# linjonathan/tropical_cyclone_risk

Hardware: AMD Instinct MI355X
Metric: storm-steps/sec (100k-storm ensemble) (higher is better)
Workload: dtype f64

## Files before the change

### tropical_cyclone_risk_amd/csrc/tcr_abi.hip

```cpp
#include <hip/hip_runtime.h>

#include <atomic>
#include <chrono>
#include <cmath>
#include <condition_variable>
#include <memory>
#include <mutex>
#include <thread>
#include <type_traits>
#include <cstdio>
#include <cstdlib>
#include <cstring>
#include <string>
#include <vector>

#include "tcr_kernels.hip"
#include "tcr_seed.hip"
#include "tcr_compact.hip"
#include "tcr_prep.hip"
#include "tcr_thermo.hip"
#ifdef TCR_EXPERIMENTS
#include "tcr_experiments.h"
#endif

// ... 136 lines not shown
    size_t vrec_cap = 0;
    unsigned long long *d_tiles = nullptr;
    size_t tiles_cap = 0;
    unsigned long long *d_queue = nullptr;
    uint16_t *d_sidx = nullptr;
    size_t sidx_cap = 0;
    double *d_park[2] = {nullptr, nullptr};
    size_t park_cap[2] = {0, 0};
    double2 *d_sc_table = nullptr;
    double *d_tab = nullptr;
    int tab_np = 0, tab_ns = 0;
    double2 *d_pf = nullptr;
    size_t pf_cap = 0;
    int fs_period = 0;
    int cu_count = 256;
    uint8_t *d_screen_skip = nullptr;
    size_t screen_skip_cap = 0;
    int32_t *d_und_list = nullptr;
    size_t und_list_cap = 0;
    unsigned long long *d_und_count = nullptr;
    float *d_stat32 = nullptr;
    bool stat32_stale = true;
    int32_t *d_tc_idx = nullptr;
    size_t tc_idx_cap = 0;
    int64_t *d_tc_count = nullptr;
    double *d_cell = nullptr; size_t cell_cap = 0; int cell_bins = 0;
    bool cell_counts_open = false;
    unsigned int *d_hist_partial = nullptr;
    uint8_t *d_probe = nullptr;
    int probe_cap = 0;
    int storms_per_lane = 1;
    tcr_tune tune;
    double *h_stage[2] = {nullptr, nullptr};
    size_t h_stage_cap = 0;
    hipEvent_t h_stage_ev[2] = {nullptr, nullptr};
// ... 578 lines not shown
template <typename R>
int integrate_impl(tcr_ctx *ctx, const tcr_storms *in, const TracksT<R> out, void *stream_, uint64_t *stats = nullptr,
                   const int64_t *stats_n_dev = nullptr, int64_t n_expected = 0)
{
    HIPCHK(ctx, hipSetDevice(ctx->device));
    const int64_t n = in->n;
    if (n < 0) return fail(ctx, "tcr_integrate: negative n");
    if (n == 0) return 0;
    hipStream_t st = stream_ ? (hipStream_t)stream_ : ctx->stream;
    const tcr_params &P = ctx->prm;
    const size_t ns = (size_t)P.n_steps;
    constexpr size_t REC = (size_t)step_rec_doubles<R>();
    if (grow(ctx, &ctx->d_fs, &ctx->fs_cap, ((size_t)n * ns * 4 * sizeof(R) + 7) / 8)) return -1;
    const int max_rk = P.max_rk_steps > 0 ? P.max_rk_steps : 64;
    if (grow(ctx, &ctx->d_srec, &ctx->srec_cap, (size_t)n * max_rk * REC)) return -1;
    if (grow(ctx, &ctx->d_vrec, &ctx->vrec_cap, (size_t)n * max_rk * kVRec)) return -1;
    if (max_rk > 65535) return fail(ctx, "tcr_params.max_rk_steps must be <= 65535");
    {
        double *p = reinterpret_cast<double *>(ctx->d_sidx);
        if (grow(ctx, &p, &ctx->sidx_cap, ((size_t)n * ns * sizeof(uint16_t) + 7) / 8)) { ctx->d_sidx = nullptr; return -1; }
        ctx->d_sidx = reinterpret_cast<uint16_t *>(p);
    }
    R *fs = reinterpret_cast<R *>(ctx->d_fs);
    EvalKT<R> EK{};
    bool affine = false;
    if (eval_k_ready<R>(ctx, EK, &affine, st)) return -1;

    hipEvent_t *ev = nullptr;
    if (ctx->timing && !ctx->capturing && timing_events(ctx, &ev)) return -1;
    if (ev) HIPCHK(ctx, hipEventRecord(ev[0], st));
    const int wps = std::is_same<R, double>::value ? TCR_INT_WPS : TCR_INT_WPS_F32;
    unsigned waves = integrate_waves(ctx, (n_expected > 0 && n_expected < n) ? n_expected : n, wps);
    const int thr = park_threshold(ctx, waves, wps);
    const unsigned final_waves = park_final_waves(ctx);
    const bool segmented = kFsMfmaColGroups == 2 && thr > 0 && waves > final_waves && kMaxPasses > 1 && fourier_on_matrix_cores(ctx) &&
                           (int)P.n_steps > kFsSegSamples + 16 && ctx->tune.table_segments != 0;
    int prune_sample = -1;
    if (out.tc_rows_only && ctx->tune.prune != 0) {
        const double t2d = 2 * 86400.0, step_out = P.total_time / (double)(P.n_steps - 1);
        const int j = (int)floor(t2d / step_out);
        if (j >= 1 && j < P.n_steps - 1 && ts_host(P, j) == t2d) {
            prune_sample = j;
            double *q = reinterpret_cast<double *>(ctx->d_screen_skip);
            if (grow(ctx, &q, &ctx->screen_skip_cap, ((size_t)n + 7) / 8)) { ctx->d_screen_skip = nullptr; return -1; }
            ctx->d_screen_skip = reinterpret_cast<uint8_t *>(q);
            double *u = reinterpret_cast<double *>(ctx->d_und_list);
            if (grow(ctx, &u, &ctx->und_list_cap, ((size_t)n + 1) / 2 + 1)) { ctx->d_und_list = nullptr; return -1; }
            ctx->d_und_list = reinterpret_cast<int32_t *>(u);
            if (!ctx->d_und_count && dev_alloc(ctx, &ctx->d_und_count, (size_t)1)) return -1;
        }
    }
    {
        BatchReset z{};
        z.queue = ctx->d_queue; z.queue_words = (int)kQueueWords;
        if (prune_sample >= 0) { z.und_count = ctx->d_und_count; z.flags = out.flags; z.n_flags = n; }
        if (out.tc_rows_only) z.tc_count = reinterpret_cast<unsigned long long *>(ctx->d_tc_count);
        if (launch_fourier<R>(ctx, n, in->n_dev, in->phases, fs, st, segmented ? kFsFirst : kFsAll, nullptr, nullptr, &z)) return -1;
    }
    STAGE(TCR_STAGE_FOURIER);
    if (ev) HIPCHK(ctx, hipEventRecord(ev[1], st));
    {
        KArgsT<R> a{};
        a.P = P; a.D = dev_fields(ctx); a.K = EK; a.n = n; a.n_dev = in->n_dev;
        a.lon0 = in->lon0; a.lat0 = in->lat0; a.v0 = in->v0; a.m0 = in->m0; a.h_bl = in->h_bl;
        a.slot = in->slot; a.phases = in->phases; a.fs = fs; a.srec = ctx->d_srec; a.vrec = ctx->d_vrec; a.max_rk_steps = max_rk;
        a.n_valid = out.n_valid; a.status = out.status; a.nfev = out.nfev;
        a.n_accept = out.n_accept; a.n_reject = out.n_reject;
        a.queue = ctx->d_queue;
        a.prune_sample = prune_sample;
        a.screen_skip = prune_sample >= 0 ? ctx->d_screen_skip : nullptr;
        if (prune_sample >= 0) {
            a.und_list = ctx->d_und_list; a.und_count = ctx->d_und_count;
        }
        const size_t park_items = segmented ? (size_t)n : (size_t)waves * kWave;
        if (thr > 0 && grow(ctx, &ctx->d_park[0], &ctx->park_cap[0], park_items * kParkRec)) return -1;
        if (thr > 0 && grow(ctx, &ctx->d_park[1], &ctx->park_cap[1], park_items * kParkRec)) return -1;
        const bool probe = std::is_same<R, double>::value && ctx->d_probe;
        if (probe) { a.probe = ctx->d_probe; a.probe_cap = ctx->probe_cap; }
        bool seg_events = false;
        for (int pass = 0; pass < kMaxPasses; ++pass) {
            const bool last = thr <= 0 || waves <= final_waves || pass == kMaxPasses - 1;
            a.pass = pass;
            a.fill_pct = pass_fill_pct();
            a.threshold = last ? 0 : thr;
            a.park_in = ctx->d_park[(pass + 1) & 1];
            a.park_out = ctx->d_park[pass & 1];
            a.t_limit = (segmented && pass == 0) ? ts_host(P, kFsSegSamples - 2) : 1e300;
// ... 2 lines not shown
            if (segmented && pass == 0) {
                if (ev) HIPCHK(ctx, hipEventRecord(ev[4], st));
                if (launch_fourier<R>(ctx, n, in->n_dev, in->phases, fs, st, kFsRest, ctx->d_park[0], ctx->d_queue + kMaxPasses)) return -1;
                if (ev) HIPCHK(ctx, hipEventRecord(ev[5], st));
                seg_events = true;
                continue;
            }
            waves = (unsigned)(((size_t)waves * (size_t)(thr - 1) + kWave - 1) / kWave);
        }
        if (ev && !seg_events) { HIPCHK(ctx, hipEventRecord(ev[4], st)); HIPCHK(ctx, hipEventRecord(ev[5], st)); }
    }
    STAGE(TCR_STAGE_INTEGRATE);
    if (ev) HIPCHK(ctx, hipEventRecord(ev[2], st));
    {
        EArgsT<R> a{};
        a.P = P; a.D = dev_fields(ctx); a.n = n; a.n_dev = in->n_dev; a.max_rk_steps = max_rk; a.srec = ctx->d_srec; a.vrec = ctx->d_vrec; a.fs = fs;
        a.slot = in->slot; a.n_valid = out.n_valid; a.status = out.status; a.n_accept = out.n_accept;
        a.lon = out.lon; a.lat = out.lat; a.v = out.v; a.m = out.m; a.vmax = out.vmax;
        a.envw = out.envw; a.flags = out.flags; a.pad_state = out.pad_state;
        a.K = EK;
        a.screen_skip = prune_sample >= 0 ? ctx->d_screen_skip : nullptr;
        if (prune_sample >= 0) { a.und_list = ctx->d_und_list; a.und_count = ctx->d_und_count; }
        const unsigned chunks = (unsigned)((ns + kPostThreads - 1) / kPostThreads);
        if (out.tc_rows_only) {
            if ((size_t)n > ctx->tc_idx_cap) {
                if (ctx->d_tc_idx) HIPCHK(ctx, hipFree(ctx->d_tc_idx));
                ctx->d_tc_idx = nullptr; ctx->tc_idx_cap = 0;
                if (dev_alloc(ctx, &ctx->d_tc_idx, (size_t)n)) return -1;
                ctx->tc_idx_cap = (size_t)n;
            }
            a.tc_list = ctx->d_tc_idx; a.tc_count = reinterpret_cast<unsigned long long *>(ctx->d_tc_count);
            hipLaunchKernelGGL(k_screen<R>, dim3((unsigned)((n + kScreenStorms - 1) / kScreenStorms)), dim3(kScreenThreads), 0, st, a);
            STAGE(TCR_STAGE_SCREEN);
            STAGE(TCR_STAGE_SELECT_TC);
            a.list = ctx->d_tc_idx; a.count = ctx->d_tc_count;
        }
        int64_t cap = kEmitGridCap;
        if (ctx->tune.emit_grid_cap > 0) cap = ctx->tune.emit_grid_cap;
        const unsigned gx = (out.tc_rows_only && n > 2 * cap) ? (unsigned)cap : (unsigned)n;
        hipLaunchKernelGGL(k_dense<R>, dim3(gx), dim3(kWave), 0, st, a, ctx->d_sidx);
        STAGE(TCR_STAGE_DENSE);
        const unsigned ex = gx;
        if (out.tc_rows_only) {
            if (affine) hipLaunchKernelGGL((k_emit<R, true, false>), dim3(ex, chunks), dim3(kPostThreads), 0, st, a, ctx->d_sidx);
            else hipLaunchKernelGGL((k_emit<R, false, false>), dim3(ex, chunks), dim3(kPostThreads), 0, st, a, ctx->d_sidx);
            if ((int64_t)ex < n) {
                a.item_base = ex;
// ... 71 lines not shown
        (void)hipFree(g->d_lon); (void)hipFree(g->d_lat); (void)hipFree(g->d_rlon); (void)hipFree(g->d_rlat);
        (void)hipFree(g->d_lon32); (void)hipFree(g->d_lat32); (void)hipFree(g->d_rlon32); (void)hipFree(g->d_rlat32);
    }
    for (auto &s : ctx->slots) { (void)hipFree(s.wind); (void)hipFree(s.thermo); (void)hipFree(s.rh); (void)hipFree(s.wind32); (void)hipFree(s.thermo32); }
    (void)hipFree(ctx->d_stat32); (void)hipFree(ctx->d_land); (void)hipFree(ctx->d_bathy); (void)hipFree(ctx->d_land32); (void)hipFree(ctx->d_bathy32);
    (void)hipFree(ctx->d_slots); (void)hipFree(ctx->d_stat); (void)hipFree(ctx->d_mask_bits); (void)hipFree(ctx->d_nstat); (void)hipFree(ctx->d_nbathy);
    (void)hipFree(ctx->d_fs); (void)hipFree(ctx->d_srec); (void)hipFree(ctx->d_vrec);
    for (auto &ev : ctx->ev_pool) if (ev) (void)hipEventDestroy(ev);
    for (auto &ev : ctx->st_pool) if (ev) (void)hipEventDestroy(ev);
    for (auto &g : ctx->graphs) { if (g.exec) (void)hipGraphExecDestroy(g.exec); if (g.graph) (void)hipGraphDestroy(g.graph); }
    (void)hipFree(ctx->d_round_key);
    ctx->hz.release(); ctx->wf.release(); ctx->ls.release();
    (void)hipFree(ctx->lf_xy); (void)hipFree(ctx->lf_bits);
    (void)hipFree(ctx->d_cl);
    for (int i = 0; i < 2; ++i) { if (ctx->h_stage[i]) (void)hipHostFree(ctx->h_stage[i]); if (ctx->h_stage_ev[i]) (void)hipEventDestroy(ctx->h_stage_ev[i]); }
    (void)hipFree(ctx->d_hist_partial); (void)hipFree(ctx->d_cell); (void)hipFree(ctx->d_tiles); (void)hipFree(ctx->d_tc_idx); (void)hipFree(ctx->d_tc_count); (void)hipFree(ctx->d_queue); (void)hipFree(ctx->d_sidx); (void)hipFree(ctx->d_park[0]); (void)hipFree(ctx->d_park[1]); (void)hipFree(ctx->d_sc_table); (void)hipFree(ctx->d_pf); (void)hipFree(ctx->d_screen_skip); (void)hipFree(ctx->d_und_list); (void)hipFree(ctx->d_und_count); (void)hipFree(ctx->d_tab);
    (void)hipStreamDestroy(ctx->stream);
    delete ctx;
    return 0;
}

int tcr_params_set(tcr_ctx *ctx, const tcr_params *p)
{
    if (!ctx || !p) return -1;
    if (p->n_series < 1 || p->n_series > TCR_MAX_SERIES) return fail(ctx, "n_series out of range");
    if (p->n_steps < 2 || p->n_steps > 4096) return fail(ctx, "n_steps must be in [2, 4096]");
    if (p->max_rk_steps < 0 || p->max_rk_steps > 4096) return fail(ctx, "max_rk_steps out of range");
    if (!(p->total_time > 0) || !(p->dt_out > 0)) return fail(ctx, "total_time and dt_out must be positive");
    ctx->prm = *p;
    ctx->have_prm = true;
    ++ctx->epoch;
// ... 1181 lines not shown
```

### tropical_cyclone_risk_amd/csrc/tcr_device.h

```cpp
#pragma once
#include <hip/hip_runtime.h>
#include <stdint.h>

#include <type_traits>

#include "../../include/tcrisk_hip.h"

#define RD(x) (x)

#ifndef TCR_FUSE
#define TCR_FUSE 1
#endif
#ifndef TCR_FAST_DIV
#define TCR_FAST_DIV 1
#endif
#ifndef TCR_FAST_SQRT
#define TCR_FAST_SQRT 1
#endif
#ifndef TCR_SHARE_COS
#define TCR_SHARE_COS 1
#endif
#ifndef TCR_FAST_POW
#define TCR_FAST_POW 1
#endif
// ... 295 lines not shown
template <typename R> struct Widths;
template <> struct Widths<double> { static constexpr int W = 2, T = 2, H = 2, F = 2; };
template <> struct Widths<float> { static constexpr int W = 4, T = 4, H = 2, F = 4; };

__device__ __forceinline__ double ts_at(const tcr_params &P, int i)
{
    return (i == P.n_steps - 1) ? P.total_time : (double)i * (P.total_time / (double)(P.n_steps - 1));
}

template <typename R>
__device__ __forceinline__ double ts_k(const EvalKT<R> &K, int i)
{
    return (i == RD(K.n_steps) - 1) ? RD(K.total_time) : (double)i * RD(K.tstep);
}

struct FsBracket {
    int lo;
    double x_lo, dx;
};

template <typename R>
__device__ __forceinline__ FsBracket fs_bracket(const EvalKT<R> &K, double t)
{
    const int ns = RD(K.n_steps);
    int idx = (int)ceil(t * RD(K.inv_tstep));
    idx = idx < 0 ? 0 : (idx > ns - 1 ? ns - 1 : idx);
    const bool dn = (idx > 0) && (ts_k(K, idx - 1) >= t);
    const bool up = !dn && (idx < ns - 1) && (ts_k(K, idx) < t);
    idx += up ? 1 : (dn ? -1 : 0);
    idx = idx < 1 ? 1 : idx;
// ... 373 lines not shown
```

### tropical_cyclone_risk_amd/csrc/tcr_kernels.hip

```cpp
#include "tcr_device.h"

namespace tcr {

template <typename R>
struct KArgsT {
    tcr_params P;
    DevFields D;
    EvalKT<R> K;
    int64_t n;
    const int64_t *n_dev;
    const double *lon0, *lat0, *v0, *m0, *h_bl;
    const int32_t *slot;
    const double *phases;
    R *fs;
    double *srec;
    int32_t *n_valid, *status, *nfev, *n_accept, *n_reject;
    unsigned long long *queue;
    int max_rk_steps;
    int pass;
    int threshold;
    int fill_pct;
    const double *park_in;
    double *park_out;
    double t_limit;
    uint8_t *probe;
    int probe_cap;
    double *vrec;
    int prune_sample;
    uint8_t *screen_skip;
    int32_t *und_list;
    unsigned long long *und_count;
};
using KArgs = KArgsT<double>;
constexpr int kVRec = 12;
constexpr int kMaxPasses = 16;
constexpr int kParkRec = 18;

__device__ __forceinline__ int64_t n_eff(int64_t n, const int64_t *n_dev)
{
    if (!n_dev) return n;
    const int64_t m = *n_dev;
    return m < n ? m : n;
}

template <typename R>
__device__ __forceinline__ void store_fs(R *__restrict__ dst, double a, double b, double c, double d)
{
    typedef typename VecT<R, 4>::type V4;
    V4 v; v[0] = (R)a; v[1] = (R)b; v[2] = (R)c; v[3] = (R)d;
    *reinterpret_cast<V4 *>(dst) = v;
}
// ... 104 lines not shown
#endif
constexpr int kFsMfmaColTiles = TCR_FS_MFMA_TILES;
#ifndef TCR_FS_MFMA_WAVES
#define TCR_FS_MFMA_WAVES 2
#endif
constexpr int kFsMfmaWaves = TCR_FS_MFMA_WAVES;
constexpr int kFsMfmaColGroups = 24 / (kFsMfmaWaves * kFsMfmaColTiles);
constexpr int kFsMfmaWgsPerCu = TCR_FS_MFMA_WPS;
static_assert(kFsMfmaColGroups * kFsMfmaWaves * kFsMfmaColTiles == 24, "column tiles per wave must be 6, 3, 2 or 1");
constexpr int kFsMfmaKSteps = 8;
constexpr int kFsMfmaMaxSamples = 24 * 16;

struct BatchReset {
    unsigned long long *queue;
    int queue_words;
    unsigned long long *und_count;
    int32_t *flags;
    int64_t n_flags;
    unsigned long long *tc_count;
};
__device__ __forceinline__ void batch_reset(const BatchReset &z, int64_t i, int64_t stride)
{
    if (!z.queue) return;
    for (int64_t k = i; k < z.queue_words; k += stride) z.queue[k] = 0ull;
    if (i == 0 && z.und_count) *z.und_count = 0ull;
    if (i == 0 && z.tc_count) *z.tc_count = 0ull;
    for (int64_t k = i; k < z.n_flags; k += stride) z.flags[k] = 0;
}
__global__ __launch_bounds__(256) void k_batch_reset(BatchReset z)
{
    batch_reset(z, (int64_t)blockIdx.x * 256 + threadIdx.x, (int64_t)gridDim.x * 256);
}

__global__ __launch_bounds__(256) void k_phase_factors_frag(tcr_params P, int64_t n, const int64_t *__restrict__ n_dev,
                                                            const double *__restrict__ phases, double *__restrict__ frag,
                                                            const int64_t *__restrict__ list, const unsigned long long *__restrict__ list_count,
                                                            BatchReset z)
{
    batch_reset(z, (int64_t)blockIdx.x * 256 + threadIdx.x, (int64_t)gridDim.x * 256);
    const int N = P.n_series;
// ... 137 lines not shown
#define A30 (44. / 45)
#define A31 (-56. / 15)
#define A32 (32. / 9)
#define A40 (19372. / 6561)
#define A41 (-25360. / 2187)
#define A42 (64448. / 6561)
#define A43 (-212. / 729)
#define A50 (9017. / 3168)
#define A51 (-355. / 33)
#define A52 (46732. / 5247)
#define A53 (49. / 176)
#define A54 (-5103. / 18656)
__device__ constexpr double RK_C[7] = {0, 1. / 5, 3. / 10, 4. / 5, 8. / 9, 1, 1};
__device__ constexpr double RK_B[6] = {35. / 384, 0, 500. / 1113, 125. / 192, -2187. / 6784, 11. / 84};
__device__ constexpr double RK_E[7] = {-71. / 57600, 0, 71. / 16695, -71. / 1920, 17253. / 339200, -22. / 525, 1. / 40};
__device__ constexpr double RK_P[7][4] = {
    {1, -8048581381. / 2820520608, 8663915743. / 2820520608, -12715105075. / 11282082432},
    {0, 0, 0, 0},
    {0, 131558114200. / 32700410799, -68118460800. / 10900136933, 87487479700. / 32700410799},
    {0, -1754552775. / 470086768, 14199869525. / 1410260304, -10690763975. / 1880347072},
    {0, 127303824393. / 49829197408, -318862633887. / 49829197408, 701980252875. / 199316789632},
    {0, -282668133. / 205662961, 2019193451. / 616988883, -1453857185. / 822651844},
    {0, 40617522. / 29380423, -110615467. / 29380423, 69997945. / 29380423}};

__device__ __forceinline__ double rms4(double a, double b, double c, double d)
{
    TCR_FP_FUSE_RK
    return qsqrt<double>(a * a + b * b + c * c + d * d) / 2.0;
}

__device__ __forceinline__ int samples_upto(const tcr_params &P, double t_emit)
{
    const int ns = P.n_steps;
    int k = (int)(t_emit / (P.total_time / (double)(ns - 1)));
    k = k < 0 ? 0 : (k > ns - 1 ? ns - 1 : k);
    while (k + 1 < ns && ts_at(P, k + 1) <= t_emit) ++k;
    while (k >= 0 && ts_at(P, k) > t_emit) --k;
    return k + 1;
// ... 38 lines not shown
    __syncthreads();
    const int ns = P.n_steps;
    const double tb = P.total_time;
    constexpr int REC = step_rec_doubles<R>();
    typedef typename VecT<R, 4>::type V4;
#define KS(j, i) Kl[((j) * 4 + (i)) * kWave + lane]

    long long sid = -1;
    int status = kRunning, nfev = 0, nacc = 0, nrej = 0, next_out = 0;
    bool active = false, fresh = false, exhausted = false, rejected = false;
    const R *wind = nullptr, *thermo = nullptr;
    const R *fs = nullptr;
    double *srec = nullptr;
    R ck_h = R(0.0);
    int cur_slot = 0;
    bool doomed = false;
    R y[4] = {0, 0, 0, 0}, f[4] = {0, 0, 0, 0}, yn[4] = {0, 0, 0, 0};
    R e[4] = {0, 0, 0, 0};
    double et = 0;
    double t = 0, h = 0, ha = 0, h_abs = 0, t_new = 0;
    R g = R(0.0);
    CornerCacheT<R> CC;
    cache_reset(CC);
    RhsPipeT<R, AFFINE, SM> PIPE;
    double etn = 0;

    auto finalize = [&]() {
        a.n_valid[sid] = next_out;
        a.status[sid] = status;
        a.nfev[sid] = (status == TCR_STATUS_GATED) ? 0 : nfev;
        a.n_accept[sid] = nacc;
        a.n_reject[sid] = nrej;
        if (a.screen_skip) a.screen_skip[sid] = doomed ? 1 : 0;
        if (a.und_list && !doomed && status != TCR_STATUS_GATED && next_out > 0)
            a.und_list[atomicAdd(a.und_count, 1ull)] = (int32_t)sid;
        active = false;
    };
    auto attempt_setup = [&]() {
        const double min_step = 10 * fabs(nextafter(t, INFINITY) - t);
        if (ha < min_step) { status = TCR_STATUS_STEP_FAIL; finalize(); return; }
        h = ha;
        t_new = t + h;
        if (t_new - tb > 0) t_new = tb;
        h = t_new - t;
        ha = fabs(h);
        for (int i = 0; i < 4; ++i) {
            KS(0, i) = f[i];
            const R dy = R(0.0) + f[i] * R(A10);
            e[i] = y[i] + dy * (R)h;
        }
// ... 5 lines not shown
        if (ha > P.max_step) ha = P.max_step;
        else if (ha < min_step) ha = min_step;
        rejected = false;
        attempt_setup();
    };

    auto park = [&](unsigned long long mask) {
        const int leader = __ffsll((long long)mask) - 1;
        unsigned long long base = 0;
        if (lane == leader) base = atomicAdd(a.queue + kMaxPasses + a.pass, (unsigned long long)__popcll(mask));
        base = __shfl(base, leader);
        if ((mask >> lane) & 1ull) {
            const size_t item = (size_t)(base + (unsigned long long)__popcll(mask & ((1ull << lane) - 1ull)));
            double2 *o = reinterpret_cast<double2 *>(a.park_out + item * kParkRec);
            const long long c0 = (long long)(unsigned)nfev | ((long long)nacc << 32);
            const long long c1 = (long long)(unsigned)nrej | ((long long)(doomed ? 1 : 0) << 30) | ((long long)(rejected ? 1 : 0) << 31) | ((long long)next_out << 32);
            o[0] = make_double2(t, h); o[1] = make_double2(t_new, ha); o[2] = make_double2((double)g, (double)y[0]);
            o[3] = make_double2((double)y[1], (double)y[2]); o[4] = make_double2((double)y[3], (double)f[0]);
            o[5] = make_double2((double)f[1], (double)f[2]);
            o[6] = make_double2((double)f[3], __longlong_as_double(sid));
            o[7] = make_double2(__longlong_as_double(c0), __longlong_as_double(c1));
            o[8] = make_double2((double)ck_h, __longlong_as_double((long long)cur_slot));
        }
    };
    __shared__ unsigned long long occ[4];
    if (lane == 0) { occ[0] = 0; occ[1] = 0; occ[2] = wall_clock64(); occ[3] = clock64(); }
    for (;;) {
        {
            const unsigned long long late = __ballot(active && t_new > a.t_limit);
            if (late) { park(late); if ((late >> lane) & 1ull) active = false; }
        }
// ... 2 lines not shown
            const int leader = __ffsll((long long)want) - 1;
            unsigned long long base = 0;
            if (lane == leader) base = atomicAdd(q_head, (unsigned long long)__popcll(want));
            base = __shfl(base, leader);
            if (!active && !exhausted) {
                const long long item = (long long)(base + (unsigned long long)__popcll(want & ((1ull << lane) - 1ull)));
                if (item >= n_items) {
                    exhausted = true;
                } else {
                    int slot_id;
                    if (a.pass == 0) {
                        sid = item;
                        const double lo0 = a.lon0[sid], la0 = a.lat0[sid], vv0 = a.v0[sid], mm0 = a.m0[sid], hb0 = a.h_bl[sid];
                        slot_id = a.slot[sid];
                        y[0] = (R)lo0; y[1] = (R)la0; y[2] = (R)vv0; y[3] = (R)mm0; ck_h = ck_over_h<R>(K, (R)hb0);
                        status = kRunning; nfev = 0; nacc = 0; nrej = 0; next_out = 0; doomed = false;
                        t = 0.0;
                        et = 0.0; e[0] = y[0]; e[1] = y[1]; e[2] = y[2]; e[3] = y[3];
                        fresh = true;
                    } else {
                        const double2 *r = reinterpret_cast<const double2 *>(a.park_in + (size_t)item * kParkRec);
                        const double2 r0 = r[0], r1 = r[1], r2 = r[2], r3 = r[3], r4 = r[4], r5 = r[5], r6 = r[6], r7 = r[7], r8 = r[8];
                        t = r0.x; h = r0.y; t_new = r1.x; ha = r1.y; g = (R)r2.x;
                        y[0] = (R)r2.y; y[1] = (R)r3.x; y[2] = (R)r3.y; y[3] = (R)r4.x;
                        f[0] = (R)r4.y; f[1] = (R)r5.x; f[2] = (R)r5.y; f[3] = (R)r6.x;
                        sid = __double_as_longlong(r6.y);
                        const long long c0 = __double_as_longlong(r7.x), c1 = __double_as_longlong(r7.y);
                        nfev = (int)(c0 & 0xffffffffll); nacc = (int)(c0 >> 32);
                        nrej = (int)(c1 & 0x3fffffffll); doomed = (c1 >> 30) & 1; rejected = (c1 >> 31) & 1; next_out = (int)(c1 >> 32);
                        ck_h = (R)r8.x; slot_id = (int)__double_as_longlong(r8.y);
                        status = kRunning;
                        for (int i = 0; i < 4; ++i) {
                            KS(0, i) = f[i];
                            const R dy = R(0.0) + f[i] * R(A10);
                            e[i] = y[i] + dy * (R)h;
                        }
                        et = t + RK_C[1] * h;
                        fresh = false;
                    }
                    if (slot_id < kIntSlotCache) { wind = s_wind[slot_id]; thermo = s_thermo[slot_id]; }
                    else { const DevSlot S = D.slots[slot_id]; wind = slot_wind<R>(S); thermo = slot_thermo<R>(S); }
                    cur_slot = slot_id;
                    fs = a.fs + sid * ns * 4;
                    srec = a.srec + sid * (long long)a.max_rk_steps * REC;
// ... 58 lines not shown
                    et = etn;
                } else {
                    double er[4];
                    for (int i = 0; i < 4; ++i) {
                        const double sc = P.atol + fmax(fabs((double)y[i]), fabs((double)yn[i])) * P.rtol;
                        double acc = 0.0;
                        for (int j = 0; j < 7; ++j) acc += (double)KS(j, i) * RK_E[j];
                        er[i] = qdiv_nz<double>(acc * h, sc);
                    }
                    const double err = rms4(er[0], er[1], er[2], er[3]);
                    const double pw = 0.9 * inv_fifth_root<double>(err);
                    if (err < 1) {
                        double fac = (err == 0) ? 10.0 : fmin(10.0, pw);
                        if (rejected && fac > 1) fac = 1;
                        ha *= fac;
                        if (nacc < a.max_rk_steps && !doomed) {
                            double *rec = srec + (size_t)nacc * REC;
                            double2 *o = reinterpret_cast<double2 *>(rec);
                            o[0] = make_double2(t, h);
                            o[1] = make_double2(t_new, 0.0);
                            V4 *body = reinterpret_cast<V4 *>(rec + kStepHdr);
                            V4 v; v[0] = y[0]; v[1] = y[1]; v[2] = y[2]; v[3] = y[3];
                            body[0] = v;
                            for (int j = 0; j < 7; ++j) {
                                V4 kk; kk[0] = KS(j, 0); kk[1] = KS(j, 1); kk[2] = KS(j, 2); kk[3] = KS(j, 3);
                                body[1 + j] = kk;
                            }
                            double2 *vr = reinterpret_cast<double2 *>(a.vrec + (sid * (long long)a.max_rk_steps + nacc) * kVRec);
                            vr[0] = make_double2(t, h);
                            vr[1] = make_double2(t_new, (double)y[2]);
                            vr[2] = make_double2((double)KS(0, 2), (double)KS(1, 2));
                            vr[3] = make_double2((double)KS(2, 2), (double)KS(3, 2));
                            vr[4] = make_double2((double)KS(4, 2), (double)KS(5, 2));
                            vr[5] = make_double2((double)KS(6, 2), 0.0);
                        }
                        ++nacc;
                        const double t_old = t;
                        t = t_new;
                        const R v_old = y[2];
                        for (int i = 0; i < 4; ++i) { y[i] = yn[i]; f[i] = r.d[i]; }
                        h_abs = ha;
                        if (t - tb >= 0) status = TCR_STATUS_FINISHED;
                        const R g_new = event_fn<R>(P, y[0], y[1], y[2]);
                        double t_emit = t;
                        if (g == R(0.0)) { status = TCR_STATUS_EVENT; t_emit = t_old; }
                        else if (g_new == R(0.0)) status = TCR_STATUS_EVENT;
                        g = g_new;
                        const int first_out = next_out;
                        next_out = samples_upto(P, t_emit);
                        int s2d = -1;
                        if (a.prune_sample >= 0 && !doomed) {
                            if (first_out <= a.prune_sample && a.prune_sample < next_out) s2d = a.prune_sample;
                            else if (status != kRunning && next_out <= a.prune_sample && first_out < next_out) s2d = next_out - 1;
                        }
                        if (s2d >= 0) {
                            TCR_FP_EXACT
                            R Qv[4];
                            for (int k = 0; k < 4; ++k) {
                                R acc = R(0.0);
                                for (int q = 0; q < 7; ++q) acc += KS(q, 2) * R(RK_P[q][k]);
                                Qv[k] = acc;
                            }
                            const R x = (R)((ts_at(P, s2d) - t_old) / h);
                            const R p1 = x, p2 = p1 * x, p3 = p2 * x, p4 = p3 * x;
                            R acc = R(0.0);
                            acc += Qv[0] * p1; acc += Qv[1] * p2; acc += Qv[2] * p3; acc += Qv[3] * p4;
                            const R v2d = (R)h * acc + v_old;
                            doomed = !((double)v2d >= P.v_2d_thresh);
                        }
                        if (status == kRunning && !doomed && nacc >= a.max_rk_steps) status = TCR_STATUS_STEP_OVERFLOW;
                        if (status != kRunning) finalize();
                        else begin_step();
                    } else {
                        ha *= fmax(0.2, pw);
                        rejected = true;
                        ++nrej;
                        attempt_setup();
                    }
                }
            } else if (live && slot == 0) {
                const R sdu = r.w[0] - r.w[2], sdw = r.w[1] - r.w[3];
                const R shear = sqrt(sdu * sdu + sdw * sdw);
                if (r.vpot > R(0) && shear * r.chi / r.vpot >= R(1)) {
                    status = TCR_STATUS_GATED;
                    finalize();
// ... 44 lines not shown
    DevFields D;
    int64_t n;
    const int64_t *n_dev;
    int max_rk_steps;
    const double *srec;
    const double *vrec;
    const R *fs;
    const int32_t *slot;
    const int32_t *n_valid, *status, *n_accept;
    R *lon, *lat, *v, *m, *vmax, *envw;
    int32_t *flags;
    const int32_t *pad_state;
    const int32_t *list;
    const int64_t *count;
    int64_t item_base;
    const uint8_t *screen_skip;
    const int32_t *und_list;
    const unsigned long long *und_count;
    int32_t *tc_list;
    unsigned long long *tc_count;
    EvalKT<R> K;
};
using EArgs = EArgsT<double>;
static_assert(sizeof(EvalKT<double>) % 8 == 0 && sizeof(EvalKT<float>) % 8 == 0, "EvalK is copied to LDS in eight-byte words");
constexpr int kBitAny15 = 1 << 8, kBitVmax = 1 << 9;
constexpr int kBitListed = 1 << 10;
#ifndef TCR_POST_THREADS
#define TCR_POST_THREADS 128
#endif
constexpr int kPostThreads = TCR_POST_THREADS;
#ifndef TCR_EMIT_GRID_CAP
#define TCR_EMIT_GRID_CAP 8192
#endif
// ... 190 lines not shown
            }
        }
    } while (LIST && (item += gridDim.x) < n_items);
}

constexpr int kScreenThreads = 256;
constexpr int kScreenGroup = 16;
constexpr int kScreenStorms = kScreenThreads / kScreenGroup;

template <typename R>
__global__ __launch_bounds__(kScreenThreads, TCR_SHADOW_WPS) void k_screen(EArgsT<R> a)
{
    __shared__ R cap[kScreenStorms][3];
    const tcr_params &P = a.P;
    const int g = threadIdx.x / kScreenGroup, l = threadIdx.x % kScreenGroup;
    const int64_t item = (int64_t)blockIdx.x * kScreenStorms + g;
    if (a.und_list && (int64_t)blockIdx.x * kScreenStorms >= (int64_t)*a.und_count) return;
    const bool listed = a.und_list && item < (int64_t)*a.und_count;
    const int64_t sid = a.und_list ? (listed ? (int64_t)a.und_list[item] : 0) : item;
    const bool on = a.und_list ? listed : sid < a.n;
    const bool exists = a.und_list ? listed : sid < n_eff(a.n, a.n_dev);
    const int ns = P.n_steps;
    int n = 0, nst = 0, st = TCR_STATUS_GATED;
    if (exists) {
        n = a.n_valid[sid]; nst = a.n_accept[sid]; st = a.status[sid];
        nst = nst < a.max_rk_steps ? nst : a.max_rk_steps;
        if (a.screen_skip && a.screen_skip[sid]) n = 0;
    }
    const double step_out = P.total_time / (double)(ns - 1);
    const double t2d = 2 * 86400.0;
    const bool clamp2d = n > 0 && t2d >= ts_at(P, n - 1);
    const int j2d = clamp2d ? n - 1 : (int)floor(t2d / step_out);
    bool any15 = false;
    const double *vrec_storm = a.vrec + sid * (int64_t)a.max_rk_steps * kVRec;
    struct StepV {
        double t_old, h64;
        R hh, y0, Q[4];
        int i_lo, i_hi;
    };
    auto load_step = [&](int j) {
        const double2 *rj = reinterpret_cast<const double2 *>(vrec_storm + (size_t)j * kVRec);
        const double2 r0 = rj[0], r1 = rj[1], r2 = rj[2], r3 = rj[3], r4 = rj[4], r5 = rj[5];
        StepV s;
        s.t_old = r0.x; s.h64 = r0.y;
        const double t_new = r1.x;
        s.hh = (R)s.h64; s.y0 = (R)r1.y;
        const R kq[7] = {(R)r2.x, (R)r2.y, (R)r3.x, (R)r3.y, (R)r4.x, (R)r4.y, (R)r5.x};
        for (int k = 0; k < 4; ++k) {
            R acc = R(0.0);
            for (int q = 0; q < 7; ++q) acc += kq[q] * R(RK_P[q][k]);
            s.Q[k] = acc;
        }
        s.i_lo = (j == 0) ? 0 : samples_upto(P, s.t_old);
        s.i_hi = samples_upto(P, t_new);
        s.i_hi = s.i_hi < n ? s.i_hi : n;
        return s;
    };
    auto v_at = [&](const StepV &s, int i) -> R {
        const R x = (R)((ts_at(P, i) - s.t_old) / s.h64);
        const R p1 = x, p2 = p1 * x, p3 = p2 * x, p4 = p3 * x;
        R acc = R(0.0);
        acc += s.Q[0] * p1; acc += s.Q[1] * p2; acc += s.Q[2] * p3; acc += s.Q[3] * p4;
        return s.hh * acc + s.y0;
    };
    auto caps = [&](const StepV &s) {
        if (s.i_lo <= j2d && j2d < s.i_hi) cap[g][0] = v_at(s, j2d);
        if (s.i_lo <= j2d + 1 && j2d + 1 < s.i_hi) cap[g][1] = v_at(s, j2d + 1);
        if (s.i_lo <= n - 1 && n - 1 < s.i_hi) cap[g][2] = v_at(s, n - 1);
    };
    const bool has0 = l < nst && n > 0;
    StepV s0{};
    if (has0) { s0 = load_step(l); caps(s0); }
    for (int j = l + kScreenGroup; j < nst && n > 0; j += kScreenGroup) caps(load_step(j));
    __syncthreads();
    bool pass2d = false;
    if (n > 0 && st != TCR_STATUS_GATED) {
        double v2d;
        if (clamp2d) v2d = (double)cap[g][2];
        else v2d = interp_v2d<R>(cap[g][0], cap[g][1], ts_at(P, j2d), ts_at(P, j2d + 1), t2d);
        pass2d = v2d >= P.v_2d_thresh;
    }
    const R thr = (R)P.v_thresh, band = sizeof(R) == 8 ? R(1e-9) : R(2e-3), margin = sizeof(R) == 8 ? R(1e-3) : R(1e-2);
    auto scan = [&](const StepV &s) {
        const R z = R(0.0);
        const R up = (s.Q[0] > z ? s.Q[0] : z) + (s.Q[1] > z ? s.Q[1] : z) + (s.Q[2] > z ? s.Q[2] : z) + (s.Q[3] > z ? s.Q[3] : z);
        const R ub = s.y0 + fabs(s.hh) * up;
        if (ub < thr - margin) return;
        const double rh = 1.0 / s.h64;
        for (int i = s.i_lo; i < s.i_hi && !any15; ++i) {
            const R x = (R)((ts_at(P, i) - s.t_old) * rh);
            const R v_f = s.hh * (x * (s.Q[0] + x * (s.Q[1] + x * (s.Q[2] + x * s.Q[3])))) + s.y0;
            bool hit = v_f >= thr + band;
            const bool amb = !hit && v_f >= thr - band;
            if (__ballot(amb)) {
                asm volatile("" ::: "memory");
                if (amb) hit = v_at(s, i) >= thr;
            }
            any15 = any15 || hit;
        }
    };
    if (pass2d) {
        if (has0) scan(s0);
        for (int j = l + kScreenGroup; j < nst; j += kScreenGroup) scan(load_step(j));
    }
    int hit = any15 ? 1 : 0;
    for (int off = kScreenGroup / 2; off > 0; off >>= 1) hit |= __shfl_xor(hit, off);
    any15 = hit != 0;
    if (on && l == 0) {
        const bool tc = any15 && pass2d;
        a.flags[sid] = tc ? TCR_FLAG_IS_TC : 0;
        if (tc && a.tc_list) a.tc_list[atomicAdd(a.tc_count, 1ull)] = (int32_t)sid;
    }
}

// ... 186 lines not shown
```

Before: 10.55 billion.

## Fuse TC screening into integrator, dropping vrec records and screen kernel

When pruning is active, the integrator now tracks the 2-day and v_thresh screening criteria inline using per-step dense-output polynomials, stored as a small bitfield that is carried through parking. Storms that qualify are appended directly to the TC list. This removes the per-step velocity record writes, the vrec buffer allocation, the separate k_screen launch, and the undecided-list machinery. The cost is extra polynomial evaluation and divergence inside the hot integrator loop, plus some risk of subtle semantic mismatch with the old post-hoc screen (for example the handling of the last sample when the run ends before day 2).

```diff
diff --git a/tropical_cyclone_risk_amd/csrc/tcr_abi.hip b/tropical_cyclone_risk_amd/csrc/tcr_abi.hip
--- a/tropical_cyclone_risk_amd/csrc/tcr_abi.hip
+++ b/tropical_cyclone_risk_amd/csrc/tcr_abi.hip
@@ -174,11 +174,6 @@
     size_t pf_cap = 0;
     int fs_period = 0;
     int cu_count = 256;
-    uint8_t *d_screen_skip = nullptr;
-    size_t screen_skip_cap = 0;
-    int32_t *d_und_list = nullptr;
-    size_t und_list_cap = 0;
-    unsigned long long *d_und_count = nullptr;
     float *d_stat32 = nullptr;
     bool stat32_stale = true;
     int32_t *d_tc_idx = nullptr;
@@ -787,7 +782,6 @@
     if (grow(ctx, &ctx->d_fs, &ctx->fs_cap, ((size_t)n * ns * 4 * sizeof(R) + 7) / 8)) return -1;
     const int max_rk = P.max_rk_steps > 0 ? P.max_rk_steps : 64;
     if (grow(ctx, &ctx->d_srec, &ctx->srec_cap, (size_t)n * max_rk * REC)) return -1;
-    if (grow(ctx, &ctx->d_vrec, &ctx->vrec_cap, (size_t)n * max_rk * kVRec)) return -1;
     if (max_rk > 65535) return fail(ctx, "tcr_params.max_rk_steps must be <= 65535");
     {
         double *p = reinterpret_cast<double *>(ctx->d_sidx);
@@ -812,21 +806,20 @@
     if (out.tc_rows_only && ctx->tune.prune != 0) {
         const double t2d = 2 * 86400.0, step_out = P.total_time / (double)(P.n_steps - 1);
         const int j = (int)floor(t2d / step_out);
-        if (j >= 1 && j < P.n_steps - 1 && ts_host(P, j) == t2d) {
-            prune_sample = j;
-            double *q = reinterpret_cast<double *>(ctx->d_screen_skip);
-            if (grow(ctx, &q, &ctx->screen_skip_cap, ((size_t)n + 7) / 8)) { ctx->d_screen_skip = nullptr; return -1; }
-            ctx->d_screen_skip = reinterpret_cast<uint8_t *>(q);
-            double *u = reinterpret_cast<double *>(ctx->d_und_list);
-            if (grow(ctx, &u, &ctx->und_list_cap, ((size_t)n + 1) / 2 + 1)) { ctx->d_und_list = nullptr; return -1; }
-            ctx->d_und_list = reinterpret_cast<int32_t *>(u);
-            if (!ctx->d_und_count && dev_alloc(ctx, &ctx->d_und_count, (size_t)1)) return -1;
-        }
+        if (j >= 1 && j < P.n_steps - 1 && ts_host(P, j) == t2d) prune_sample = j;
+    }
+    const bool in_flight = prune_sample >= 0;
+    if (!in_flight && grow(ctx, &ctx->d_vrec, &ctx->vrec_cap, (size_t)n * max_rk * kVRec)) return -1;
+    if (out.tc_rows_only && (size_t)n > ctx->tc_idx_cap) {
+        if (ctx->d_tc_idx) HIPCHK(ctx, hipFree(ctx->d_tc_idx));
+        ctx->d_tc_idx = nullptr; ctx->tc_idx_cap = 0;
+        if (dev_alloc(ctx, &ctx->d_tc_idx, (size_t)n)) return -1;
+        ctx->tc_idx_cap = (size_t)n;
     }
     {
         BatchReset z{};
         z.queue = ctx->d_queue; z.queue_words = (int)kQueueWords;
-        if (prune_sample >= 0) { z.und_count = ctx->d_und_count; z.flags = out.flags; z.n_flags = n; }
+        if (in_flight) { z.flags = out.flags; z.n_flags = n; }
         if (out.tc_rows_only) z.tc_count = reinterpret_cast<unsigned long long *>(ctx->d_tc_count);
         if (launch_fourier<R>(ctx, n, in->n_dev, in->phases, fs, st, segmented ? kFsFirst : kFsAll, nullptr, nullptr, &z)) return -1;
     }
@@ -836,14 +829,13 @@
         KArgsT<R> a{};
         a.P = P; a.D = dev_fields(ctx); a.K = EK; a.n = n; a.n_dev = in->n_dev;
         a.lon0 = in->lon0; a.lat0 = in->lat0; a.v0 = in->v0; a.m0 = in->m0; a.h_bl = in->h_bl;
-        a.slot = in->slot; a.phases = in->phases; a.fs = fs; a.srec = ctx->d_srec; a.vrec = ctx->d_vrec; a.max_rk_steps = max_rk;
+        a.slot = in->slot; a.phases = in->phases; a.fs = fs; a.srec = ctx->d_srec; a.vrec = in_flight ? nullptr : ctx->d_vrec; a.max_rk_steps = max_rk;
         a.n_valid = out.n_valid; a.status = out.status; a.nfev = out.nfev;
         a.n_accept = out.n_accept; a.n_reject = out.n_reject;
         a.queue = ctx->d_queue;
         a.prune_sample = prune_sample;
-        a.screen_skip = prune_sample >= 0 ? ctx->d_screen_skip : nullptr;
-        if (prune_sample >= 0) {
-            a.und_list = ctx->d_und_list; a.und_count = ctx->d_und_count;
+        if (in_flight) {
+            a.tc_list = ctx->d_tc_idx; a.tc_count = reinterpret_cast<unsigned long long *>(ctx->d_tc_count);
         }
         const size_t park_items = segmented ? (size_t)n : (size_t)waves * kWave;
         if (thr > 0 && grow(ctx, &ctx->d_park[0], &ctx->park_cap[0], park_items * kParkRec)) return -1;
@@ -876,23 +868,17 @@
     if (ev) HIPCHK(ctx, hipEventRecord(ev[2], st));
     {
         EArgsT<R> a{};
-        a.P = P; a.D = dev_fields(ctx); a.n = n; a.n_dev = in->n_dev; a.max_rk_steps = max_rk; a.srec = ctx->d_srec; a.vrec = ctx->d_vrec; a.fs = fs;
+        a.P = P; a.D = dev_fields(ctx); a.n = n; a.n_dev = in->n_dev; a.max_rk_steps = max_rk; a.srec = ctx->d_srec; a.vrec = in_flight ? nullptr : ctx->d_vrec; a.fs = fs;
         a.slot = in->slot; a.n_valid = out.n_valid; a.status = out.status; a.n_accept = out.n_accept;
         a.lon = out.lon; a.lat = out.lat; a.v = out.v; a.m = out.m; a.vmax = out.vmax;
         a.envw = out.envw; a.flags = out.flags; a.pad_state = out.pad_state;
         a.K = EK;
-        a.screen_skip = prune_sample >= 0 ? ctx->d_screen_skip : nullptr;
-        if (prune_sample >= 0) { a.und_list = ctx->d_und_list; a.und_count = ctx->d_und_count; }
         const unsigned chunks = (unsigned)((ns + kPostThreads - 1) / kPostThreads);
         if (out.tc_rows_only) {
-            if ((size_t)n > ctx->tc_idx_cap) {
-                if (ctx->d_tc_idx) HIPCHK(ctx, hipFree(ctx->d_tc_idx));
-                ctx->d_tc_idx = nullptr; ctx->tc_idx_cap = 0;
-                if (dev_alloc(ctx, &ctx->d_tc_idx, (size_t)n)) return -1;
-                ctx->tc_idx_cap = (size_t)n;
+            if (!in_flight) {
+                a.tc_list = ctx->d_tc_idx; a.tc_count = reinterpret_cast<unsigned long long *>(ctx->d_tc_count);
+                hipLaunchKernelGGL(k_screen<R>, dim3((unsigned)((n + kScreenStorms - 1) / kScreenStorms)), dim3(kScreenThreads), 0, st, a);
             }
-            a.tc_list = ctx->d_tc_idx; a.tc_count = reinterpret_cast<unsigned long long *>(ctx->d_tc_count);
-            hipLaunchKernelGGL(k_screen<R>, dim3((unsigned)((n + kScreenStorms - 1) / kScreenStorms)), dim3(kScreenThreads), 0, st, a);
             STAGE(TCR_STAGE_SCREEN);
             STAGE(TCR_STAGE_SELECT_TC);
             a.list = ctx->d_tc_idx; a.count = ctx->d_tc_count;
@@ -994,7 +980,7 @@
     (void)hipFree(ctx->lf_xy); (void)hipFree(ctx->lf_bits);
     (void)hipFree(ctx->d_cl);
     for (int i = 0; i < 2; ++i) { if (ctx->h_stage[i]) (void)hipHostFree(ctx->h_stage[i]); if (ctx->h_stage_ev[i]) (void)hipEventDestroy(ctx->h_stage_ev[i]); }
-    (void)hipFree(ctx->d_hist_partial); (void)hipFree(ctx->d_cell); (void)hipFree(ctx->d_tiles); (void)hipFree(ctx->d_tc_idx); (void)hipFree(ctx->d_tc_count); (void)hipFree(ctx->d_queue); (void)hipFree(ctx->d_sidx); (void)hipFree(ctx->d_park[0]); (void)hipFree(ctx->d_park[1]); (void)hipFree(ctx->d_sc_table); (void)hipFree(ctx->d_pf); (void)hipFree(ctx->d_screen_skip); (void)hipFree(ctx->d_und_list); (void)hipFree(ctx->d_und_count); (void)hipFree(ctx->d_tab);
+    (void)hipFree(ctx->d_hist_partial); (void)hipFree(ctx->d_cell); (void)hipFree(ctx->d_tiles); (void)hipFree(ctx->d_tc_idx); (void)hipFree(ctx->d_tc_count); (void)hipFree(ctx->d_queue); (void)hipFree(ctx->d_sidx); (void)hipFree(ctx->d_park[0]); (void)hipFree(ctx->d_park[1]); (void)hipFree(ctx->d_sc_table); (void)hipFree(ctx->d_pf); (void)hipFree(ctx->d_tab);
     (void)hipStreamDestroy(ctx->stream);
     delete ctx;
     return 0;
diff --git a/tropical_cyclone_risk_amd/csrc/tcr_device.h b/tropical_cyclone_risk_amd/csrc/tcr_device.h
--- a/tropical_cyclone_risk_amd/csrc/tcr_device.h
+++ b/tropical_cyclone_risk_amd/csrc/tcr_device.h
@@ -333,6 +333,71 @@
     return (i == RD(K.n_steps) - 1) ? RD(K.total_time) : (double)i * RD(K.tstep);
 }
 
+__device__ constexpr double RK_P[7][4] = {
+    {1, -8048581381. / 2820520608, 8663915743. / 2820520608, -12715105075. / 11282082432},
+    {0, 0, 0, 0},
+    {0, 131558114200. / 32700410799, -68118460800. / 10900136933, 87487479700. / 32700410799},
+    {0, -1754552775. / 470086768, 14199869525. / 1410260304, -10690763975. / 1880347072},
+    {0, 127303824393. / 49829197408, -318862633887. / 49829197408, 701980252875. / 199316789632},
+    {0, -282668133. / 205662961, 2019193451. / 616988883, -1453857185. / 822651844},
+    {0, 40617522. / 29380423, -110615467. / 29380423, 69997945. / 29380423}};
+
+template <typename R>
+struct StepVT {
+    double t_old, h64;
+    R hh, y0, Q[4];
+    int i_lo, i_hi;
+};
+
+template <typename R>
+__device__ __forceinline__ void dense_v_row(const R (&kq)[7], R (&Q)[4])
+{
+    TCR_FP_EXACT
+    for (int k = 0; k < 4; ++k) {
+        R acc = R(0.0);
+        for (int q = 0; q < 7; ++q) acc += kq[q] * R(RK_P[q][k]);
+        Q[k] = acc;
+    }
+}
+
+template <typename R>
+__device__ __forceinline__ R dense_v_at(const tcr_params &P, const StepVT<R> &s, int i)
+{
+    TCR_FP_EXACT
+    const R x = (R)((ts_at(P, i) - s.t_old) / s.h64);
+    const R p1 = x, p2 = p1 * x, p3 = p2 * x, p4 = p3 * x;
+    R acc = R(0.0);
+    acc += s.Q[0] * p1; acc += s.Q[1] * p2; acc += s.Q[2] * p3; acc += s.Q[3] * p4;
+    return s.hh * acc + s.y0;
+}
+
+template <typename R>
+__device__ __forceinline__ bool dense_v_below(const StepVT<R> &s, R thr)
+{
+    TCR_FP_EXACT
+    const R margin = sizeof(R) == 8 ? R(1e-3) : R(1e-2);
+    const R z = R(0.0);
+    const R up = (s.Q[0] > z ? s.Q[0] : z) + (s.Q[1] > z ? s.Q[1] : z) + (s.Q[2] > z ? s.Q[2] : z) + (s.Q[3] > z ? s.Q[3] : z);
+    const R ub = s.y0 + fabs(s.hh) * up;
+    return ub < thr - margin;
+}
+
+template <typename R>
+__device__ __forceinline__ bool dense_v_hit(const tcr_params &P, const StepVT<R> &s, double rh, R thr, int i)
+{
+    TCR_FP_EXACT
+    const R band = sizeof(R) == 8 ? R(1e-9) : R(2e-3);
+    const R x = (R)((ts_at(P, i) - s.t_old) * rh);
+    const R v_f = s.hh * (x * (s.Q[0] + x * (s.Q[1] + x * (s.Q[2] + x * s.Q[3])))) + s.y0;
+    bool hit = v_f >= thr + band;
+    const bool amb = !hit && v_f >= thr - band;
+    if (__ballot(amb)) {
+        asm volatile("" ::: "memory");
+        if (amb) hit = dense_v_at<R>(P, s, i) >= thr;
+    }
+    return hit;
+}
+
 struct FsBracket {
     int lo;
     double x_lo, dx;
diff --git a/tropical_cyclone_risk_amd/csrc/tcr_kernels.hip b/tropical_cyclone_risk_amd/csrc/tcr_kernels.hip
--- a/tropical_cyclone_risk_amd/csrc/tcr_kernels.hip
+++ b/tropical_cyclone_risk_amd/csrc/tcr_kernels.hip
@@ -27,14 +27,18 @@
     int probe_cap;
     double *vrec;
     int prune_sample;
-    uint8_t *screen_skip;
-    int32_t *und_list;
-    unsigned long long *und_count;
+    int32_t *tc_list;
+    unsigned long long *tc_count;
 };
 using KArgs = KArgsT<double>;
 constexpr int kVRec = 12;
 constexpr int kMaxPasses = 16;
 constexpr int kParkRec = 18;
+constexpr int kScrAny15 = 1;
+constexpr int kScrLastOk = 2;
+constexpr int kScrPassed = 4;
+constexpr int kScrFailed = 8;
+constexpr int kScrMask = 15, kScrShift = 27;
 
 __device__ __forceinline__ int64_t n_eff(int64_t n, const int64_t *n_dev)
 {
@@ -169,7 +173,6 @@
 struct BatchReset {
     unsigned long long *queue;
     int queue_words;
-    unsigned long long *und_count;
     int32_t *flags;
     int64_t n_flags;
     unsigned long long *tc_count;
@@ -178,7 +181,6 @@
 {
     if (!z.queue) return;
     for (int64_t k = i; k < z.queue_words; k += stride) z.queue[k] = 0ull;
-    if (i == 0 && z.und_count) *z.und_count = 0ull;
     if (i == 0 && z.tc_count) *z.tc_count = 0ull;
     for (int64_t k = i; k < z.n_flags; k += stride) z.flags[k] = 0;
 }
@@ -346,14 +348,6 @@
 __device__ constexpr double RK_C[7] = {0, 1. / 5, 3. / 10, 4. / 5, 8. / 9, 1, 1};
 __device__ constexpr double RK_B[6] = {35. / 384, 0, 500. / 1113, 125. / 192, -2187. / 6784, 11. / 84};
 __device__ constexpr double RK_E[7] = {-71. / 57600, 0, 71. / 16695, -71. / 1920, 17253. / 339200, -22. / 525, 1. / 40};
-__device__ constexpr double RK_P[7][4] = {
-    {1, -8048581381. / 2820520608, 8663915743. / 2820520608, -12715105075. / 11282082432},
-    {0, 0, 0, 0},
-    {0, 131558114200. / 32700410799, -68118460800. / 10900136933, 87487479700. / 32700410799},
-    {0, -1754552775. / 470086768, 14199869525. / 1410260304, -10690763975. / 1880347072},
-    {0, 127303824393. / 49829197408, -318862633887. / 49829197408, 701980252875. / 199316789632},
-    {0, -282668133. / 205662961, 2019193451. / 616988883, -1453857185. / 822651844},
-    {0, 40617522. / 29380423, -110615467. / 29380423, 69997945. / 29380423}};
 
 __device__ __forceinline__ double rms4(double a, double b, double c, double d)
 {
@@ -422,7 +416,7 @@
     double *srec = nullptr;
     R ck_h = R(0.0);
     int cur_slot = 0;
-    bool doomed = false;
+    int scr = 0;
     R y[4] = {0, 0, 0, 0}, f[4] = {0, 0, 0, 0}, yn[4] = {0, 0, 0, 0};
     R e[4] = {0, 0, 0, 0};
     double et = 0;
@@ -439,9 +433,9 @@
         a.nfev[sid] = (status == TCR_STATUS_GATED) ? 0 : nfev;
         a.n_accept[sid] = nacc;
         a.n_reject[sid] = nrej;
-        if (a.screen_skip) a.screen_skip[sid] = doomed ? 1 : 0;
-        if (a.und_list && !doomed && status != TCR_STATUS_GATED && next_out > 0)
-            a.und_list[atomicAdd(a.und_count, 1ull)] = (int32_t)sid;
+        if (a.tc_list && status != TCR_STATUS_GATED && next_out > 0 && (scr & kScrAny15) &&
+            ((scr & kScrPassed) || (!(scr & kScrFailed) && (scr & kScrLastOk))))
+            a.tc_list[atomicAdd(a.tc_count, 1ull)] = (int32_t)sid;
         active = false;
     };
     auto attempt_setup = [&]() {
@@ -477,7 +471,7 @@
             const size_t item = (size_t)(base + (unsigned long long)__popcll(mask & ((1ull << lane) - 1ull)));
             double2 *o = reinterpret_cast<double2 *>(a.park_out + item * kParkRec);
             const long long c0 = (long long)(unsigned)nfev | ((long long)nacc << 32);
-            const long long c1 = (long long)(unsigned)nrej | ((long long)(doomed ? 1 : 0) << 30) | ((long long)(rejected ? 1 : 0) << 31) | ((long long)next_out << 32);
+            const long long c1 = (long long)(unsigned)nrej | ((long long)scr << kScrShift) | ((long long)(rejected ? 1 : 0) << 31) | ((long long)next_out << 32);
             o[0] = make_double2(t, h); o[1] = make_double2(t_new, ha); o[2] = make_double2((double)g, (double)y[0]);
             o[3] = make_double2((double)y[1], (double)y[2]); o[4] = make_double2((double)y[3], (double)f[0]);
             o[5] = make_double2((double)f[1], (double)f[2]);
@@ -510,7 +504,7 @@
                         const double lo0 = a.lon0[sid], la0 = a.lat0[sid], vv0 = a.v0[sid], mm0 = a.m0[sid], hb0 = a.h_bl[sid];
                         slot_id = a.slot[sid];
                         y[0] = (R)lo0; y[1] = (R)la0; y[2] = (R)vv0; y[3] = (R)mm0; ck_h = ck_over_h<R>(K, (R)hb0);
-                        status = kRunning; nfev = 0; nacc = 0; nrej = 0; next_out = 0; doomed = false;
+                        status = kRunning; nfev = 0; nacc = 0; nrej = 0; next_out = 0; scr = 0;
                         t = 0.0;
                         et = 0.0; e[0] = y[0]; e[1] = y[1]; e[2] = y[2]; e[3] = y[3];
                         fresh = true;
@@ -523,7 +517,7 @@
                         sid = __double_as_longlong(r6.y);
                         const long long c0 = __double_as_longlong(r7.x), c1 = __double_as_longlong(r7.y);
                         nfev = (int)(c0 & 0xffffffffll); nacc = (int)(c0 >> 32);
-                        nrej = (int)(c1 & 0x3fffffffll); doomed = (c1 >> 30) & 1; rejected = (c1 >> 31) & 1; next_out = (int)(c1 >> 32);
+                        nrej = (int)(c1 & ((1ll << kScrShift) - 1)); scr = (int)(c1 >> kScrShift) & kScrMask; rejected = (c1 >> 31) & 1; next_out = (int)(c1 >> 32);
                         ck_h = (R)r8.x; slot_id = (int)__double_as_longlong(r8.y);
                         status = kRunning;
                         for (int i = 0; i < 4; ++i) {
@@ -612,7 +606,8 @@
                         double fac = (err == 0) ? 10.0 : fmin(10.0, pw);
                         if (rejected && fac > 1) fac = 1;
                         ha *= fac;
-                        if (nacc < a.max_rk_steps && !doomed) {
+                        const bool recorded = nacc < a.max_rk_steps && !(scr & kScrFailed);
+                        if (recorded) {
                             double *rec = srec + (size_t)nacc * REC;
                             double2 *o = reinterpret_cast<double2 *>(rec);
                             o[0] = make_double2(t, h);
@@ -624,13 +619,15 @@
                                 V4 kk; kk[0] = KS(j, 0); kk[1] = KS(j, 1); kk[2] = KS(j, 2); kk[3] = KS(j, 3);
                                 body[1 + j] = kk;
                             }
-                            double2 *vr = reinterpret_cast<double2 *>(a.vrec + (sid * (long long)a.max_rk_steps + nacc) * kVRec);
-                            vr[0] = make_double2(t, h);
-                            vr[1] = make_double2(t_new, (double)y[2]);
-                            vr[2] = make_double2((double)KS(0, 2), (double)KS(1, 2));
-                            vr[3] = make_double2((double)KS(2, 2), (double)KS(3, 2));
-                            vr[4] = make_double2((double)KS(4, 2), (double)KS(5, 2));
-                            vr[5] = make_double2((double)KS(6, 2), 0.0);
+                            if (a.vrec) {
+                                double2 *vr = reinterpret_cast<double2 *>(a.vrec + (sid * (long long)a.max_rk_steps + nacc) * kVRec);
+                                vr[0] = make_double2(t, h);
+                                vr[1] = make_double2(t_new, (double)y[2]);
+                                vr[2] = make_double2((double)KS(0, 2), (double)KS(1, 2));
+                                vr[3] = make_double2((double)KS(2, 2), (double)KS(3, 2));
+                                vr[4] = make_double2((double)KS(4, 2), (double)KS(5, 2));
+                                vr[5] = make_double2((double)KS(6, 2), 0.0);
+                            }
                         }
                         ++nacc;
                         const double t_old = t;
@@ -646,27 +643,29 @@
                         g = g_new;
                         const int first_out = next_out;
                         next_out = samples_upto(P, t_emit);
-                        int s2d = -1;
-                        if (a.prune_sample >= 0 && !doomed) {
-                            if (first_out <= a.prune_sample && a.prune_sample < next_out) s2d = a.prune_sample;
-                            else if (status != kRunning && next_out <= a.prune_sample && first_out < next_out) s2d = next_out - 1;
+                        const bool emits = first_out < next_out;
+                        const bool need2d = emits && !(scr & kScrPassed) && first_out <= a.prune_sample;
+                        const bool need15 = emits && !(scr & kScrAny15);
+                        if (a.tc_list && recorded && (need2d || need15)) {
+                            StepVT<R> sv;
+                            sv.t_old = t_old; sv.h64 = h; sv.hh = (R)h; sv.y0 = v_old; sv.i_lo = first_out; sv.i_hi = next_out;
+                            const R kq[7] = {KS(0, 2), KS(1, 2), KS(2, 2), KS(3, 2), KS(4, 2), KS(5, 2), KS(6, 2)};
+                            dense_v_row<R>(kq, sv.Q);
+                            if (need2d) {
+                                const bool at2d = a.prune_sample < next_out;
+                                const bool ok = (double)dense_v_at<R>(P, sv, at2d ? a.prune_sample : next_out - 1) >= P.v_2d_thresh;
+                                if (at2d) scr |= ok ? kScrPassed : kScrFailed;
+                                else scr = ok ? (scr | kScrLastOk) : (scr & ~kScrLastOk);
+                            }
+                            const bool reach = need15 && !(scr & kScrFailed) && !dense_v_below<R>(sv, (R)P.v_thresh);
+                            if (__ballot(reach)) {
+                                const double rh = 1.0 / h;
+                                bool hit = !reach;
+                                for (int i = sv.i_lo; i < sv.i_hi && !hit; ++i) hit = dense_v_hit<R>(P, sv, rh, (R)P.v_thresh, i);
+                                if (reach && hit) scr |= kScrAny15;
+                            }
                         }
-                        if (s2d >= 0) {
-                            TCR_FP_EXACT
-                            R Qv[4];
-                            for (int k = 0; k < 4; ++k) {
-                                R acc = R(0.0);
-                                for (int q = 0; q < 7; ++q) acc += KS(q, 2) * R(RK_P[q][k]);
-                                Qv[k] = acc;
-                            }
-                            const R x = (R)((ts_at(P, s2d) - t_old) / h);
-                            const R p1 = x, p2 = p1 * x, p3 = p2 * x, p4 = p3 * x;
-                            R acc = R(0.0);
-                            acc += Qv[0] * p1; acc += Qv[1] * p2; acc += Qv[2] * p3; acc += Qv[3] * p4;
-                            const R v2d = (R)h * acc + v_old;
-                            doomed = !((double)v2d >= P.v_2d_thresh);
-                        }
-                        if (status == kRunning && !doomed && nacc >= a.max_rk_steps) status = TCR_STATUS_STEP_OVERFLOW;
+                        if (status == kRunning && !(scr & kScrFailed) && nacc >= a.max_rk_steps) status = TCR_STATUS_STEP_OVERFLOW;
                         if (status != kRunning) finalize();
                         else begin_step();
                     } else {
@@ -741,9 +740,6 @@
     const int32_t *list;
     const int64_t *count;
     int64_t item_base;
-    const uint8_t *screen_skip;
-    const int32_t *und_list;
-    const unsigned long long *und_count;
     int32_t *tc_list;
     unsigned long long *tc_count;
     EvalKT<R> K;
@@ -964,18 +960,14 @@
     __shared__ R cap[kScreenStorms][3];
     const tcr_params &P = a.P;
     const int g = threadIdx.x / kScreenGroup, l = threadIdx.x % kScreenGroup;
-    const int64_t item = (int64_t)blockIdx.x * kScreenStorms + g;
-    if (a.und_list && (int64_t)blockIdx.x * kScreenStorms >= (int64_t)*a.und_count) return;
-    const bool listed = a.und_list && item < (int64_t)*a.und_count;
-    const int64_t sid = a.und_list ? (listed ? (int64_t)a.und_list[item] : 0) : item;
-    const bool on = a.und_list ? listed : sid < a.n;
-    const bool exists = a.und_list ? listed : sid < n_eff(a.n, a.n_dev);
+    const int64_t sid = (int64_t)blockIdx.x * kScreenStorms + g;
+    const bool on = sid < a.n;
+    const bool exists = sid < n_eff(a.n, a.n_dev);
     const int ns = P.n_steps;
     int n = 0, nst = 0, st = TCR_STATUS_GATED;
     if (exists) {
         n = a.n_valid[sid]; nst = a.n_accept[sid]; st = a.status[sid];
         nst = nst < a.max_rk_steps ? nst : a.max_rk_steps;
-        if (a.screen_skip && a.screen_skip[sid]) n = 0;
     }
     const double step_out = P.total_time / (double)(ns - 1);
     const double t2d = 2 * 86400.0;
@@ -983,11 +975,7 @@
     const int j2d = clamp2d ? n - 1 : (int)floor(t2d / step_out);
     bool any15 = false;
     const double *vrec_storm = a.vrec + sid * (int64_t)a.max_rk_steps * kVRec;
-    struct StepV {
-        double t_old, h64;
-        R hh, y0, Q[4];
-        int i_lo, i_hi;
-    };
+    typedef StepVT<R> StepV;
     auto load_step = [&](int j) {
         const double2 *rj = reinterpret_cast<const double2 *>(vrec_storm + (size_t)j * kVRec);
         const double2 r0 = rj[0], r1 = rj[1], r2 = rj[2], r3 = rj[3], r4 = rj[4], r5 = rj[5];
@@ -996,23 +984,13 @@
         const double t_new = r1.x;
         s.hh = (R)s.h64; s.y0 = (R)r1.y;
         const R kq[7] = {(R)r2.x, (R)r2.y, (R)r3.x, (R)r3.y, (R)r4.x, (R)r4.y, (R)r5.x};
-        for (int k = 0; k < 4; ++k) {
-            R acc = R(0.0);
-            for (int q = 0; q < 7; ++q) acc += kq[q] * R(RK_P[q][k]);
-            s.Q[k] = acc;
-        }
+        dense_v_row<R>(kq, s.Q);
         s.i_lo = (j == 0) ? 0 : samples_upto(P, s.t_old);
         s.i_hi = samples_upto(P, t_new);
         s.i_hi = s.i_hi < n ? s.i_hi : n;
         return s;
     };
-    auto v_at = [&](const StepV &s, int i) -> R {
-        const R x = (R)((ts_at(P, i) - s.t_old) / s.h64);
-        const R p1 = x, p2 = p1 * x, p3 = p2 * x, p4 = p3 * x;
-        R acc = R(0.0);
-        acc += s.Q[0] * p1; acc += s.Q[1] * p2; acc += s.Q[2] * p3; acc += s.Q[3] * p4;
-        return s.hh * acc + s.y0;
-    };
+    auto v_at = [&](const StepV &s, int i) -> R { return dense_v_at<R>(P, s, i); };
     auto caps = [&](const StepV &s) {
         if (s.i_lo <= j2d && j2d < s.i_hi) cap[g][0] = v_at(s, j2d);
         if (s.i_lo <= j2d + 1 && j2d + 1 < s.i_hi) cap[g][1] = v_at(s, j2d + 1);
@@ -1030,24 +1008,11 @@
         else v2d = interp_v2d<R>(cap[g][0], cap[g][1], ts_at(P, j2d), ts_at(P, j2d + 1), t2d);
         pass2d = v2d >= P.v_2d_thresh;
     }
-    const R thr = (R)P.v_thresh, band = sizeof(R) == 8 ? R(1e-9) : R(2e-3), margin = sizeof(R) == 8 ? R(1e-3) : R(1e-2);
+    const R thr = (R)P.v_thresh;
     auto scan = [&](const StepV &s) {
-        const R z = R(0.0);
-        const R up = (s.Q[0] > z ? s.Q[0] : z) + (s.Q[1] > z ? s.Q[1] : z) + (s.Q[2] > z ? s.Q[2] : z) + (s.Q[3] > z ? s.Q[3] : z);
-        const R ub = s.y0 + fabs(s.hh) * up;
-        if (ub < thr - margin) return;
+        if (dense_v_below<R>(s, thr)) return;
         const double rh = 1.0 / s.h64;
-        for (int i = s.i_lo; i < s.i_hi && !any15; ++i) {
-            const R x = (R)((ts_at(P, i) - s.t_old) * rh);
-            const R v_f = s.hh * (x * (s.Q[0] + x * (s.Q[1] + x * (s.Q[2] + x * s.Q[3])))) + s.y0;
-            bool hit = v_f >= thr + band;
-            const bool amb = !hit && v_f >= thr - band;
-            if (__ballot(amb)) {
-                asm volatile("" ::: "memory");
-                if (amb) hit = v_at(s, i) >= thr;
-            }
-            any15 = any15 || hit;
-        }
+        for (int i = s.i_lo; i < s.i_hi && !any15; ++i) any15 = any15 || dense_v_hit<R>(P, s, rh, thr, i);
     };
     if (pass2d) {
         if (has0) scan(s0);
```

Result: faster. 10.80 billion (median of 6 runs) (+2.4%).
